# arnaucube/fhe-study

Measured on AMD Instinct MI355X. Metric: NTT/s (N=2^16, 64-bit q) per node; achieved HBM GB/s vs roofline, higher is better.
Workload: dtype u64

## Files before the change

### fhe-study_amd/binding.py

```python
import ctypes
import os
import subprocess
import sys

import numpy as np

_HERE = os.path.dirname(os.path.abspath(__file__))
LIB_PATH = os.environ.get("FHE_NTT_LIB") or os.path.join(_HERE, "libfhe_ntt.so")
CSRC = os.path.join(_HERE, "csrc")
SOURCES = ["capi.hip", "ntt_kernels.hip", "ntt_kernels_q62.hip", "ntt_persist.hip", "digit_mac.hip", "digit32.hip", "bfv32.hip", "smallq.hip", "generic63.hip", "zring.hip", "glue.hip", "tfhe_boot.hip"]
HEADERS = ["ntt_kernels.hpp", "ntt_rounds.hpp", "ntt_persist.hpp", "persist_sched.hpp", "digit_mac.hpp", "digit32.hpp", "bfv32.hpp", "smallq.hpp", "ntt32_rounds.hpp", "ntt32_big.hpp", "zq_device.hpp", "capi_internal.hpp", "mac_kernel.hpp", "ntt_kernels.hip",
           os.path.join("..", "..", "include", "fhe_ntt.h"), os.path.join("..", "..", "include", "fhe_ntt_experimental.h")]
OBJ_DIR = os.path.join(_HERE, "build")
HIPCC_FLAGS = ["--offload-arch=gfx950", "-O3", "-std=c++17", "-fPIC", "-Wno-unused-result",
               "-ffp-contract=off"]

FHE_OK = 0
FHE_E_BAD_N = -1
FHE_E_BAD_Q = -2
FHE_E_NO_ROOT = -3
FHE_E_NULL = -4
FHE_E_HIP = -5
FHE_E_NO_DEVICE = -6
FHE_E_PARAM_MISMATCH = -7
FHE_E_NOT_CANONICAL = -8
FHE_E_INVALID = -9
FHE_A_IS_EVALS, FHE_B_IS_EVALS, FHE_OUT_EVALS = 1, 2, 4

EXPORTS = [
    "fhe_ntt_plan_get", "fhe_ntt_plan_info", "fhe_ntt_plan_tables",
    "fhe_ntt_forward", "fhe_ntt_inverse", "fhe_rq_mul", "fhe_rq_mul_checked",
    "fhe_rq_pointwise_mul", "fhe_rq_check_canonical",
    "fhe_ntt_forward_dev", "fhe_ntt_inverse_dev", "fhe_rq_mul_dev",
    "fhe_rq_mul_workspace_bytes", "fhe_rq_pointwise_mul_dev", "fhe_fill_synthetic_dev",
    "fhe_ntt_set_batch_tile", "fhe_ntt_kernel_timing_enable", "fhe_ntt_kernel_timing_read",
    "fhe_ntt_kernel_timing_reset",
    "fhe_ntt_device_count", "fhe_last_error", "fhe_ntt_version", "fhe_ntt_shutdown",
    "fhe_ntt_plan_prepare", "fhe_ntt_plan_arithmetic", "fhe_ntt_set_check_canonical", "fhe_shard_range", "fhe_shard_gather_dev", "fhe_ntt_release_stream_workspace", "fhe_ntt_workspace_bytes",
    "fhe_tggsw_prepared_words", "fhe_tggsw_prepare_dev", "fhe_tggsw_external_product_prepared_dev",
    "fhe_glwe_ksk_prepared_words", "fhe_glwe_ksk_prepare_dev", "fhe_glwe_key_switch_prepared_dev",
    "fhe_bfv_rlk_prepared_words", "fhe_bfv_rlk_prepare_dev", "fhe_bfv_relinearize_prepared_dev", "fhe_bfv_mul_prepared_dev",
    "fhe_r_naive_mul", "fhe_r_naive_mul_dev", "fhe_mul_div_round_dev",
    "fhe_bfv_tensor", "fhe_bfv_tensor_dev", "fhe_bfv_relinearize_dev", "fhe_bfv_mul", "fhe_bfv_mul_dev",
    "fhe_tn_mul", "fhe_tn_mul_dev", "fhe_tggsw_external_product", "fhe_tggsw_external_product_dev",
# ... 561 lines not shown
```

### fhe-study_amd/csrc/bfv32.hip

```cpp
#include "bfv32.hpp"
#include "ntt32_big.hpp"

#include <type_traits>

namespace fhe {

__device__ __forceinline__ u32 mont32(u32 x, u32 y, u32 p, u32 pinv_neg) {
    const u64 t = (u64)x * y;
    const u32 m = (u32)t * pinv_neg;
    return (u32)((t + (u64)m * p) >> 32);
}
__device__ __forceinline__ u64 crt2(u32 rA, u32 rB, u32 pA, u32 pB, Tw32 crt) {
    const u32 rAb = csub_u32(rA, pB);
    const u32 diff = rB - rAb + pB;
    const u32 h = csub_u32(mul_shoup32(diff, crt, pB), pB);
    return (u64)rA + (u64)pA * h;
}

#ifndef FHE_B32_INV_T
#define FHE_B32_INV_T 2
#endif
#ifndef FHE_B32_INV_R
#define FHE_B32_INV_R 1
#endif
#ifndef FHE_B32_FWD_PRELOAD
#define FHE_B32_FWD_PRELOAD 1
#endif
#ifndef FHE_B32_FWD_WAVES
#define FHE_B32_FWD_WAVES 4
#endif
#ifndef FHE_B32_RELIN_WAVES
#define FHE_B32_RELIN_WAVES 4
#endif
#ifndef FHE_B32_FWD2_WAVES
#define FHE_B32_FWD2_WAVES 6
#endif
#ifndef FHE_B32_FWD2_PRELOAD
#define FHE_B32_FWD2_PRELOAD 0
#endif
#ifndef FHE_B32_FWD3_WAVES
#define FHE_B32_FWD3_WAVES 4
#endif
#ifndef FHE_B32_FWD3_RELOAD
#define FHE_B32_FWD3_RELOAD 0
#endif
constexpr int fwd_waves(int npr) { return npr == 2 ? FHE_B32_FWD2_WAVES : npr == 3 ? FHE_B32_FWD3_WAVES : FHE_B32_FWD_WAVES; }
constexpr bool fwd_reload(int npr) { return npr == 3 && FHE_B32_FWD3_RELOAD != 0; }
constexpr bool fwd_preload(int npr) { return npr == 2 ? FHE_B32_FWD2_PRELOAD != 0 : FHE_B32_FWD_PRELOAD != 0; }
#ifndef FHE_B32_PARK_LDS
#define FHE_B32_PARK_LDS 1
#endif
constexpr int kRelinWps = 4;
#ifndef FHE_B32_INV_LOOSE
#define FHE_B32_INV_LOOSE 1
#endif
template <int MODE> constexpr int last_in_of() { return (FHE_B32_INV_LOOSE && MODE != 0) ? 8 : 2; }
template <int MODE, int LB>
__device__ __forceinline__ void inv_block(u32 (&v)[1][16], u32 *lds, const Tw32 *ltw, const Tw32 *gtw, u32 tf, u32 p, u32 p2, u32 bq, u32 blk) {
    if constexpr (FHE_B32_INV_LOOSE && MODE != 0) inv_big_loose<LB, MODE == 2, last_in_of<MODE>()>(v, lds, ltw, gtw, tf, p, bq, 1u, blk);
    else if constexpr (MODE == 0) inv_big<LB>(v, lds, ltw, gtw, tf, p, p2, 1u, blk);
    else if constexpr (MODE == 1) inv_big_direct<LB, false>(v, lds, ltw, gtw, tf, p, p2, 1u, blk);
    else inv_big_direct<LB, true>(v, lds, ltw, gtw, tf, p, p2, 1u, blk);
}
template <int LB>
struct Blk {
    using C = Big32<LB>;
    static constexpr u32 M = C::M, TH = C::TH;
    static constexpr size_t LDS(int tables) { return C::TILE_BYTES + (size_t)tables * C::TW_BYTES; }
    static constexpr int park_lds(int tables, int words, int wps) {
        const long wgs = (4L * wps * 64) / (long)TH;
        const long budget = 160L * 1024 / (wgs < 1 ? 1 : wgs) - 1024;
        const long k = (budget - (long)LDS(tables)) / (8L * (long)TH);
        return k < 0 ? 0 : (k > words ? words : (int)k);
    }
    static constexpr size_t LDS_PARKED(int tables, int words, int wps) { return LDS(tables) + (size_t)park_lds(tables, words, wps) * 8 * TH; }
    static __device__ __forceinline__ Tw32 *table(unsigned char *smem, int i) { return reinterpret_cast<Tw32 *>(smem + C::TILE_BYTES + i * C::TW_BYTES); }
};

template <int LB, int NPR, bool WORD32, bool BELOWP = false>
__global__ __launch_bounds__((Big32<LB>::TH), fwd_waves(NPR)) void bfv32_forward_kernel(Bfv32Args a) {
    static_assert(!BELOWP || WORD32, "words below a 27-bit prime are below 2^32");
    using C = Big32<LB>;
    using K = Blk<LB>;
    extern __shared__ __attribute__((aligned(16))) unsigned char smem_raw[];
    u32 *lds = reinterpret_cast<u32 *>(smem_raw);
    const u32 tf = threadIdx.x;
    const u64 g8 = blockIdx.x / 16;
    const u32 r16 = blockIdx.x % 16;
    const u64 row = g8 * 8 + (r16 & 7u);
    const u32 blk = r16 >> 3;
    if (row >= a.rows) return;
#pragma unroll
    for (int i = 0; i < NPR; i++) stage_tw32_block<C::TH>(K::table(smem_raw, i), a.t.tw_fwd[NPR == 1 ? blockIdx.y : i], C::LTW_N, tf, 1u, blk);
    const u64 *__restrict__ src = a.src + row * K::M;
    typename std::conditional<WORD32, u32, u64>::type x[16];
#pragma unroll
    for (int k = 0; k < 16; k++) x[k] = (typename std::conditional<WORD32, u32, u64>::type)src[(u32)k * C::TH + tf];
    __syncthreads();
#pragma unroll
    for (int i = 0; i < NPR; i++) {
        const u32 pr = NPR == 1 ? blockIdx.y : (u32)i;
        const u32 p = a.t.p[pr], p2 = 2u * p;
        if constexpr (fwd_reload(NPR)) {
            if (i > 0) {
                u64 sa = reinterpret_cast<u64>(src);
                asm volatile("" : "+s"(sa));
                const gu64 *ps = reinterpret_cast<const gu64 *>(sa);
#pragma unroll
                for (int k = 0; k < 16; k++) x[k] = (typename std::conditional<WORD32, u32, u64>::type)ps[(u32)k * C::TH + tf];
            }
        }
        u32 v[1][16];
#pragma unroll
        for (int k = 0; k < 16; k++)
            v[0][k] = BELOWP ? (u32)x[k] : WORD32 ? csub_u32(barrett2p_32((u32)x[k], p, a.t.bq[pr]), p) : reduce64_32(x[k], p, a.t.mu[pr]);
        fwd_big<LB, 0, 1, fwd_preload(NPR)>(v, lds, K::table(smem_raw, i), a.t.tw_fwd[pr], tf, p, p2, a.t.bq[pr], 1u, blk);
        u32 *__restrict__ dst = a.fw + (((u64)pr * a.rows + row) << (LB + 1)) + blk * K::M + tf * 4u;
#pragma unroll
        for (int j = 0; j < 4; j++) {
            uint4 o;
            o.x = barrett2p_32(v[0][4 * j], p, a.t.bq[pr]); o.y = barrett2p_32(v[0][4 * j + 1], p, a.t.bq[pr]);
            o.z = barrett2p_32(v[0][4 * j + 2], p, a.t.bq[pr]); o.w = barrett2p_32(v[0][4 * j + 3], p, a.t.bq[pr]);
            *reinterpret_cast<uint4 *>(dst + j * (K::M / 4)) = o;
// ... 30 lines not shown

#ifndef FHE_B32_INT_TAIL
#define FHE_B32_INT_TAIL 1
#endif
__device__ __forceinline__ u64 zq_from_f64_small(double ef, double qf, double qinv, u32 q) {
    const double e = round(ef);
#if FHE_B32_INT_TAIL
    const double k = floor(e * qinv);
    int r = (int)fma(-k, qf, e);
    r += (r >> 31) & (int)q;
    return (u64)min((u32)r, (u32)r - q);
#else
    const double k = rint(e * qinv);
    double r = fma(-k, qf, e);
    r = r < 0.0 ? r + qf : r;
    r = r < 0.0 ? r + qf : r;
    r = r >= qf ? r - qf : r;
    return (u64)(u32)r;
#endif
}
__device__ __forceinline__ double exact_quotient(double N, double den, double rden) {
    const double q0 = N * rden;
    const double r = fma(-q0, den, N);
    return fma(r, rden, q0);
}
template <bool SMALL>
__device__ __forceinline__ u64 scale_round(const Bfv32Args &a, long long v) {
    const double N = a.numf * (double)v;
    const double x = a.rdenf != 0.0 ? exact_quotient(N, a.denf, a.rdenf) : N / a.denf;
    if constexpr (SMALL) return zq_from_f64_small(x, (double)a.q, a.qinvf, (u32)a.q);
    else return zq_from_f64_mu(a.q, a.qmu, round(x));
}

template <int LB, bool INT, bool SMALL>
__global__ __launch_bounds__((Big32<LB>::TH), 4) void bfv32_tensor_inverse_kernel(Bfv32Args a) {
    using C = Big32<LB>;
    using K = Blk<LB>;
    extern __shared__ __attribute__((aligned(16))) unsigned char smem_raw[];
    u32 *lds = reinterpret_cast<u32 *>(smem_raw);
    const u32 tf = threadIdx.x;
    const u64 g8 = blockIdx.x / 24;
    const u32 r24 = blockIdx.x % 24;
    const u64 b = g8 * 8 + (r24 & 7u);
    const u32 which = r24 >> 3;
    if (b >= a.batch) return;
#pragma unroll
    for (int i = 0; i < 4; i++) stage_tw32_block<C::TH>(K::table(smem_raw, i), a.t.tw_inv[i >> 1], C::LTW_N, tf, 1u, (u32)(i & 1));
    __syncthreads();
    auto prime = [&](auto prc) __attribute__((always_inline)) {
        constexpr int pr = decltype(prc)::value;
        const u32 p = a.t.p[pr], p2 = 2u * p, pn = a.pinv_neg[pr];
        const u32 *__restrict__ fw = a.fw + (((u64)pr * a.rows) << (LB + 1));
        auto block = [&](u32 blk, u32 (&v)[1][16]) __attribute__((always_inline)) {
            const u32 off = blk * K::M + tf * 4u;
            auto rowp = [&](u32 w) { return fw + (((u64)w * a.batch + b) << (LB + 1)) + off; };
            const u32 *__restrict__ ra = rowp(which == 2 ? 1 : 0), *__restrict__ rb = rowp(which == 0 ? 2 : 3);
            const u32 *__restrict__ rc = rowp(1), *__restrict__ rd = rowp(2);
#pragma unroll
            for (int j = 0; j < 4; j++) {
                const uint4 xa = *reinterpret_cast<const uint4 *>(ra + j * (K::M / 4)), xb = *reinterpret_cast<const uint4 *>(rb + j * (K::M / 4));
                u32 t[4] = {mont32(xa.x, xb.x, p, pn), mont32(xa.y, xb.y, p, pn), mont32(xa.z, xb.z, p, pn), mont32(xa.w, xb.w, p, pn)};
                if (which == 1) {
                    const uint4 xc = *reinterpret_cast<const uint4 *>(rc + j * (K::M / 4)), xd = *reinterpret_cast<const uint4 *>(rd + j * (K::M / 4));
                    t[0] = csub_u32(t[0] + mont32(xc.x, xd.x, p, pn), p2); t[1] = csub_u32(t[1] + mont32(xc.y, xd.y, p, pn), p2);
                    t[2] = csub_u32(t[2] + mont32(xc.z, xd.z, p, pn), p2); t[3] = csub_u32(t[3] + mont32(xc.w, xd.w, p, pn), p2);
                }
                v[0][4 * j] = t[0]; v[0][4 * j + 1] = t[1]; v[0][4 * j + 2] = t[2]; v[0][4 * j + 3] = t[3];
            }
#ifndef FHE_B32_ABLATE_INV
            inv_block<FHE_B32_INV_T, LB>(v, lds, K::table(smem_raw, 2 * pr + (int)blk), a.t.tw_inv[pr], tf, p, p2, a.t.bq[pr], blk);
#endif
        };
        u32 v0[1][16], v1[1][16];
        block(0u, v0);
        block(1u, v1);
        const Tw32 ni = a.ninv_mont[pr], w1ni = a.w1ninv_mont[pr];
        u64 parked = 0;
        u32 tfe = tf;
        asm volatile("" : "+v"(tfe));
        u64 *po = a.out + ((u64)which * a.batch + b) * K::M + tfe;
        u64 psa = reinterpret_cast<u64>(po);
        asm volatile("" : "+v"(psa));
        const gu64 *ps = reinterpret_cast<const gu64 *>(psa);
        if constexpr (pr == 1) parked = ps[0];
#pragma unroll
        for (int k = 0; k < 16; k++) {
            u32 rl = v0[0][k], rh = v1[0][k];
            last_stage<last_in_of<FHE_B32_INV_T>()>(rl, rh, ni, w1ni, p);
            if constexpr (pr == 0) {
                po[(u32)k * C::TH] = ((u64)rh << 32) | rl;
            } else {
                const u32 loA = (u32)parked, hiA = (u32)(parked >> 32);
                if (k + 1 < 16) parked = ps[(u32)(k + 1) * C::TH];
                const long long lo = (long long)crt2(loA, rl, a.t.p[0], a.t.p[1], a.t.crt);
                const long long hi = (long long)crt2(hiA, rh, a.t.p[0], a.t.p[1], a.t.crt);
#ifndef FHE_B32_ABLATE_EPI
                u64 zl, zh;
                if constexpr (INT) {
                    zl = zq_scale_round_int(a.int_num * (u64)lo, a.q, a.qmu);
                    zh = zq_scale_round_int(a.int_num * (u64)hi, a.q, a.qmu);
                } else {
                    zl = scale_round<SMALL>(a, lo);
                    zh = scale_round<SMALL>(a, hi);
                }
#else
                const u64 zl = (u64)lo, zh = (u64)hi;
#endif
                po[(u32)k * C::TH] = zl >= zh ? zl - zh : (a.q + zl) - zh;
                __builtin_amdgcn_sched_barrier(0);
            }
        }
    };
    prime(std::integral_constant<int, 0>{});
    prime(std::integral_constant<int, 1>{});
}

template <int LB, bool SMALL>
__global__ __launch_bounds__((Big32<LB>::TH), FHE_B32_RELIN_WAVES) void bfv32_relin_inverse_kernel(Bfv32Args a) {
    using C = Big32<LB>;
    using K = Blk<LB>;
    extern __shared__ __attribute__((aligned(16))) unsigned char smem_raw[];
    u32 *lds = reinterpret_cast<u32 *>(smem_raw);
    const u32 tf = threadIdx.x;
    const u64 g8 = blockIdx.x / 16;
    const u32 r16 = blockIdx.x % 16;
    const u64 b = g8 * 8 + (r16 & 7u);
    const u32 o = r16 >> 3;
    if (b >= a.batch) return;
#pragma unroll
    for (int i = 0; i < 6; i++) stage_tw32_block<C::TH>(K::table(smem_raw, i), a.t.tw_inv[i >> 1], C::LTW_N, tf, 1u, (u32)(i & 1));
    __syncthreads();
    const u64 off = ((u64)o * a.batch + b) * K::M + tf;
    u64 *park0 = a.park + off, *park1 = park0 + 2 * a.batch * K::M;
    auto prime = [&](auto prc) __attribute__((always_inline)) {
        constexpr int pr = decltype(prc)::value;
        const u32 p = a.t.p[pr], p2 = 2u * p, pn = a.pinv_neg[pr];
        auto block = [&](u32 blk, u32 (&v)[1][16]) __attribute__((always_inline)) {
            const u32 bo = blk * K::M + tf * 4u;
            const u32 *__restrict__ rx = a.x + (((u64)pr * a.batch + b) << (LB + 1)) + bo;
            const u32 *__restrict__ rk = a.key + (((u64)pr * 2 + o) << (LB + 1)) + bo;
#pragma unroll
            for (int j = 0; j < 4; j++) {
                const uint4 xa = *reinterpret_cast<const uint4 *>(rx + j * (K::M / 4)), xb = *reinterpret_cast<const uint4 *>(rk + j * (K::M / 4));
                v[0][4 * j] = mont32(xa.x, xb.x, p, pn); v[0][4 * j + 1] = mont32(xa.y, xb.y, p, pn);
                v[0][4 * j + 2] = mont32(xa.z, xb.z, p, pn); v[0][4 * j + 3] = mont32(xa.w, xb.w, p, pn);
            }
#ifndef FHE_B32_ABLATE_INV
            inv_block<FHE_B32_INV_R, LB>(v, lds, K::table(smem_raw, 2 * pr + (int)blk), a.t.tw_inv[pr], tf, p, p2, a.t.bq[pr], blk);
#endif
        };
        u32 v0[1][16], v1[1][16];
        block(0u, v0);
        block(1u, v1);
        const Tw32 ni = a.ninv_mont[pr], w1ni = a.w1ninv_mont[pr];
        u64 pk0 = 0, pk1 = 0;
        u64 psa0 = reinterpret_cast<u64>(park0), psa1 = reinterpret_cast<u64>(park1);
        asm volatile("" : "+v"(psa0), "+v"(psa1));
        const gu64 *ps0 = reinterpret_cast<const gu64 *>(psa0), *ps1 = reinterpret_cast<const gu64 *>(psa1);
        constexpr int KL = FHE_B32_PARK_LDS ? K::park_lds(6, 16, kRelinWps) : 0;
        u64 *lpark = reinterpret_cast<u64 *>(smem_raw + K::LDS(6)) + tf;
// ... 56 lines not shown
bool bfv32_shape_supported(uint64_t q, uint64_t n, uint64_t pq) {
    if (n < 1024 || n > 8192 || (n & (n - 1)) || q < 2) return false;
    const unsigned ln = bits_of64(n - 1), bq = bits_of64(q - 1);
    if (2 * bq + ln + 1 > 54) return false;
    if (pq && (pq < q || bq + bits_of64(pq - 1) + ln > 82)) return false;
    return true;
}

template <typename K>
static hipError_t launch_big(K kernel, const char *name, int lp, size_t lds, unsigned th, u64 grid, const Bfv32Args &a, hipStream_t st,
                             unsigned gridy = 1) {
    if (grid == 0) return hipSuccess;
    if (grid > 0x7fffffffull) return hipErrorInvalidValue;
    if (hipError_t e = allow_big_lds((const void *)kernel, lds)) return e;
    KernelTimer kt(name, lp, st);
    hipLaunchKernelGGL(kernel, dim3((unsigned)grid, gridy), dim3(th), lds, st, a);
    return hipGetLastError();
}
#define FHE_BIG_SWITCH(KERNEL, NAME, GRID, GRIDY, TABLES, PARKW, WPS)                                                               \
    switch (a.log_n2) {                                                                                                      \
        case 11: return launch_big(KERNEL<10>, NAME, 11, Blk<10>::LDS_PARKED(TABLES, PARKW, WPS), Big32<10>::TH, GRID, a, st, GRIDY); \
        case 12: return launch_big(KERNEL<11>, NAME, 12, Blk<11>::LDS_PARKED(TABLES, PARKW, WPS), Big32<11>::TH, GRID, a, st, GRIDY); \
        case 13: return launch_big(KERNEL<12>, NAME, 13, Blk<12>::LDS_PARKED(TABLES, PARKW, WPS), Big32<12>::TH, GRID, a, st, GRIDY); \
        case 14: return launch_big(KERNEL<13>, NAME, 14, Blk<13>::LDS_PARKED(TABLES, PARKW, WPS), Big32<13>::TH, GRID, a, st, GRIDY); \
    }                                                                                                                        \
    return hipErrorNotSupported;

template <int LB> static constexpr auto bfv32_forward2 = bfv32_forward_kernel<LB, 2, true>;
template <int LB> static constexpr auto bfv32_forward3 = bfv32_forward_kernel<LB, 3, true>;
template <int LB> static constexpr auto bfv32_forward2b = bfv32_forward_kernel<LB, 2, true, true>;
template <int LB> static constexpr auto bfv32_forward3b = bfv32_forward_kernel<LB, 3, true, true>;
template <int LB> static constexpr auto bfv32_forward1w = bfv32_forward_kernel<LB, 1, false>;
hipError_t launch_bfv32_forward(const Bfv32Args &a, hipStream_t st) {
    const u64 grid = 16 * ((a.rows + 7) / 8);
    if (a.primes == 2 && a.word32 && a.below_p) { FHE_BIG_SWITCH(bfv32_forward2b, "bfv32_forward", grid, 1, 2, 0, 4) }
    if (a.primes == 3 && a.word32 && a.below_p) { FHE_BIG_SWITCH(bfv32_forward3b, "bfv32_forward3", grid, 1, 3, 0, 4) }
    if (a.primes == 2 && a.word32) { FHE_BIG_SWITCH(bfv32_forward2, "bfv32_forward", grid, 1, 2, 0, 4) }
    if (a.primes == 3 && a.word32) { FHE_BIG_SWITCH(bfv32_forward3, "bfv32_forward3", grid, 1, 3, 0, 4) }
    if (a.primes == 3) { FHE_BIG_SWITCH(bfv32_forward1w, "bfv32_forward_key", grid, 3, 1, 0, 4) }
    return hipErrorNotSupported;
}
template <int LB> static constexpr auto bfv32_tensor_inverse_f64 = bfv32_tensor_inverse_kernel<LB, false, false>;
template <int LB> static constexpr auto bfv32_tensor_inverse_f64s = bfv32_tensor_inverse_kernel<LB, false, true>;
template <int LB> static constexpr auto bfv32_tensor_inverse_int = bfv32_tensor_inverse_kernel<LB, true, false>;
hipError_t launch_bfv32_tensor_inverse(const Bfv32Args &a, hipStream_t st) {
    if (a.int_num) { FHE_BIG_SWITCH(bfv32_tensor_inverse_int, "bfv32_tensor_inverse", 24 * ((a.batch + 7) / 8), 1, 4, 0, 4) }
    if (a.small_f64) { FHE_BIG_SWITCH(bfv32_tensor_inverse_f64s, "bfv32_tensor_inverse", 24 * ((a.batch + 7) / 8), 1, 4, 0, 4) }
    FHE_BIG_SWITCH(bfv32_tensor_inverse_f64, "bfv32_tensor_inverse", 24 * ((a.batch + 7) / 8), 1, 4, 0, 4)
}
template <int LB> static constexpr auto bfv32_relin_inverse_gen = bfv32_relin_inverse_kernel<LB, false>;
template <int LB> static constexpr auto bfv32_relin_inverse_small = bfv32_relin_inverse_kernel<LB, true>;
hipError_t launch_bfv32_relin_inverse(const Bfv32Args &a, hipStream_t st) {
    if (a.small_f64) { FHE_BIG_SWITCH(bfv32_relin_inverse_small, "bfv32_relin_inverse", 16 * ((a.batch + 7) / 8), 1, 6, (FHE_B32_PARK_LDS ? 16 : 0), kRelinWps) }
    FHE_BIG_SWITCH(bfv32_relin_inverse_gen, "bfv32_relin_inverse", 16 * ((a.batch + 7) / 8), 1, 6, (FHE_B32_PARK_LDS ? 16 : 0), kRelinWps)
}
#undef FHE_BIG_SWITCH

bool bfv32_ablated() {
#if defined(FHE_B32_ABLATE_INV) || defined(FHE_B32_ABLATE_EPI)
    return true;
#else
    return false;
#endif
}

}
```

### fhe-study_amd/csrc/bfv32.hpp

```cpp
#pragma once
#include "digit32.hpp"

namespace fhe {

struct Bfv32Args {
    Ext32Args t;
    uint32_t pinv_neg[3];
    Tw32 ninv_mont[3];
    Tw32 w1ninv_mont[3];
    uint32_t log_n2;
    const u64 *src;
    uint32_t *fw;
    u64 rows;
    uint32_t primes;
    uint32_t word32;
    uint32_t below_p;
    const uint32_t *x, *key;
    const u64 *addend;
    u64 *out;
    u64 *park;
    u64 batch, q;
    u64 qmu;
    double numf, denf;
    double rdenf;
    u64 int_num;
    uint32_t small_f64;
    double qinvf;
};

bool bfv32_shape_supported(uint64_t q, uint64_t n, uint64_t pq);
hipError_t launch_bfv32_forward(const Bfv32Args &a, hipStream_t st);
hipError_t launch_bfv32_tensor_inverse(const Bfv32Args &a, hipStream_t st);
hipError_t launch_bfv32_relin_inverse(const Bfv32Args &a, hipStream_t st);

}
```

### fhe-study_amd/csrc/zring.hip

```cpp
#include <cstdio>
#include <cstdlib>
#include <cstring>
#include <map>
#include <vector>

#include "capi_internal.hpp"
#include "digit_mac.hpp"
#include "digit32.hpp"
#include "bfv32.hpp"
#include "ntt_rounds.hpp"
#include "zq_device.hpp"
#include "mac_kernel.hpp"

using fhe::Mod;
using fhe::Tw;
using fhe::u32;
using fhe::u64;
typedef unsigned __int128 u128;

static const u64 kCrtPrimes[3] = {
    2305843009211596801ull,
    2305843009196916737ull,
    2305843009146585089ull,
};
// ... 443 lines not shown

static bool bfv32_on(uint64_t q, uint64_t n, uint64_t pq) { return fhe_ext32_enabled() && fhe::bfv32_shape_supported(q, n, pq); }
static int bfv32_args(uint64_t n, fhe::Bfv32Args *a) {
    int rc = fhe_ext32_tables(2 * n, &a->t);
    if (rc != FHE_OK) return rc;
    a->log_n2 = ceil_log2(2 * n);
    for (int i = 0; i < 3; i++) {
        const uint32_t p = a->t.p[i];
        uint32_t inv = p;
        for (int it = 0; it < 5; it++) inv *= 2u - p * inv;
        a->pinv_neg[i] = 0u - inv;
        const u64 w = ((u64)a->t.ninv[i].w << 32) % p;
        a->ninv_mont[i] = fhe::Tw32{(uint32_t)w, (uint32_t)((w << 32) / p)};
        const fhe_ntt_plan *plan = nullptr;
        if ((rc = fhe_ntt_plan_get(p, 2 * n, &plan)) != FHE_OK) return rc;
        const u64 w1 = (plan->roots_inv[1] * w) % p;
        a->w1ninv_mont[i] = fhe::Tw32{(uint32_t)w1, (uint32_t)((w1 << 32) / p)};
    }
    return FHE_OK;
}
static bool bfv32_small_f64_on() {
    static const bool on = [] { const char *e = getenv("FHE_BFV_SMALL_F64"); return !(e && e[0] == '0'); }();
    return on;
}
static double bfv32_rden(uint64_t den) {
    static const bool on = [] { const char *e = getenv("FHE_BFV_FAST_DIV"); return !(e && e[0] == '0'); }();
    return (on && (den & 1ull) && den < (1ull << 48)) ? 1.0 / (double)den : 0.0;
}
static uint32_t bfv32_below_p(uint64_t q, const fhe::Bfv32Args &a, int primes) {
    static const bool on = [] { const char *e = getenv("FHE_BFV_BELOW_P"); return !(e && e[0] == '0'); }();
    for (int i = 0; i < primes; i++) if (q > a.t.p[i]) return 0u;
    return on ? 1u : 0u;
}
static int bfv32_tensor(uint64_t q, uint64_t n, uint64_t t, const void *d_ab, void *d_c, size_t batch, hipStream_t st) {
    fhe::Bfv32Args a{};
    int rc = bfv32_args(n, &a);
    if (rc != FHE_OK) return rc;
    void *wsv = nullptr;
    if ((rc = fhe_workspace_get(1, (u64)2 * 4 * batch * 2 * n * 4, st, &wsv)) != FHE_OK) return rc;
    a.src = (const u64 *)d_ab; a.fw = (uint32_t *)wsv; a.rows = 4 * (u64)batch; a.primes = 2; a.word32 = 1;
    a.below_p = bfv32_below_p(q, a, 2);
    if (a.below_p && (rc = fhe_check_canonical_words(q, d_ab, 4 * batch * n, st, "fhe_bfv_tensor_dev")) != FHE_OK) return rc;
    hipError_t e = fhe::launch_bfv32_forward(a, st);
    if (e != hipSuccess) return fhe_hip_fail(e, "bfv32_forward_kernel");
    a.batch = batch; a.out = (u64 *)d_c; a.q = q; a.qmu = ~0ull / q; a.numf = (double)t; a.denf = (double)q;
    a.rdenf = ((unsigned __int128)2 * n * (q - 1) * (q - 1) * t / q < ((unsigned __int128)1 << 52)) ? bfv32_rden(q) : 0.0;
    {
        static const bool on = [] { const char *e = getenv("FHE_BFV_INT_ROUND"); return e && e[0] == '1'; }();
        const unsigned __int128 vmax = (unsigned __int128)2 * n * (q - 1) * (q - 1);
        a.int_num = (on && t != 0 && vmax * t < ((unsigned __int128)1 << 52)) ? t : 0;
        a.small_f64 = (bfv32_small_f64_on() && q < (1ull << 30) && vmax * t / q < ((unsigned __int128)1 << 50)) ? 1u : 0u;
        a.qinvf = 1.0 / (double)q;
    }
    e = fhe::launch_bfv32_tensor_inverse(a, st);
    return e == hipSuccess ? FHE_OK : fhe_hip_fail(e, "bfv32_tensor_inverse_kernel");
}
static int bfv32_rlk_prepare(uint64_t n, const u64 *d_rlk, void *prep, hipStream_t st) {
    fhe::Bfv32Args a{};
    int rc = bfv32_args(n, &a);
    if (rc != FHE_OK) return rc;
    a.src = d_rlk; a.fw = (uint32_t *)prep; a.rows = 2; a.primes = 3;
    hipError_t e = fhe::launch_bfv32_forward(a, st);
    return e == hipSuccess ? FHE_OK : fhe_hip_fail(e, "bfv32_forward_kernel");
}
static int bfv32_relinearize(uint64_t q, uint64_t n, uint64_t pq, const void *d_prep, const void *d_c, void *d_out, size_t batch,
                             hipStream_t st) {
    fhe::Bfv32Args a{};
    int rc = bfv32_args(n, &a);
    if (rc != FHE_OK) return rc;
    void *wsv = nullptr;
    const u64 x_bytes = (u64)3 * batch * 2 * n * 4, park_bytes = (u64)2 * 2 * batch * n * 8;
    if ((rc = fhe_workspace_get(1, x_bytes + park_bytes, st, &wsv)) != FHE_OK) return rc;
    a.park = (u64 *)((unsigned char *)wsv + x_bytes);
    a.src = (const u64 *)d_c + 2 * (u64)batch * n; a.fw = (uint32_t *)wsv; a.rows = batch; a.primes = 3; a.word32 = 1;
    a.below_p = bfv32_below_p(q, a, 3);
    if (a.below_p && (rc = fhe_check_canonical_words(q, a.src, batch * n, st, "fhe_bfv_relinearize_dev (c2)")) != FHE_OK) return rc;
    hipError_t e = fhe::launch_bfv32_forward(a, st);
    if (e != hipSuccess) return fhe_hip_fail(e, "bfv32_forward_kernel");
    a.x = (const uint32_t *)wsv; a.key = (const uint32_t *)d_prep;
    a.addend = (const u64 *)d_c; a.out = (u64 *)d_out; a.batch = batch; a.q = q; a.qmu = ~0ull / q; a.numf = 1.0; a.denf = (double)(pq / q);
    a.rdenf = (pq % q == 0 && pq / q >= (1ull << 12)) ? bfv32_rden(pq / q) : 0.0;
    a.small_f64 = (bfv32_small_f64_on() && q < (1ull << 30) && pq / q >= (1ull << 14)) ? 1u : 0u;
    a.qinvf = 1.0 / (double)q;
    e = fhe::launch_bfv32_relin_inverse(a, st);
    return e == hipSuccess ? FHE_OK : fhe_hip_fail(e, "bfv32_relin_inverse_kernel");
}

extern "C" int fhe_bfv_tensor_dev(uint64_t q, uint64_t n, uint64_t t, const void *d_ab, void *d_c, size_t batch,
                                  void *hip_stream) {
    int rc = check_pow2_n(n, "fhe_bfv_tensor_dev");
    if (rc != FHE_OK) return rc;
    if (q < 2 || (q >> 63)) return fhe_fail(FHE_E_BAD_Q, "fhe_bfv_tensor_dev: q must be in [2, 2^63)");
    if (batch == 0) return FHE_OK;
    if (!d_ab || !d_c) return fhe_fail(FHE_E_NULL, "fhe_bfv_tensor_dev: NULL buffer");
    REQUIRE_ALIGNED(d_ab); REQUIRE_ALIGNED(d_c);
    if (bfv32_on(q, n, 0)) return bfv32_tensor(q, n, t, d_ab, d_c, batch, (hipStream_t)hip_stream);
    const u64 n2 = 2 * n;
    ZCtx z;
    rc = zctx_init(&z, n2, primes_for_bits(2 * bits_of(q - 1) + ceil_log2(n) + 1, false));
    if (rc != FHE_OK) return rc;
    hipStream_t st = (hipStream_t)hip_stream;
    const u64 words = batch * n2;
    void *wsv = nullptr;
    rc = fhe_workspace_get(1, (4 + 3 * (size_t)z.K) * words * 8, st, &wsv);
    if (rc != FHE_OK) return rc;
    u64 *AB = (u64 *)wsv, *R = AB + 4 * words;
    for (int k = 0; k < z.K; k++) {
        if ((rc = z_forward_src(z, k, (const u64 *)d_ab, AB, 4 * batch, n, st)) != FHE_OK) return rc;
        u64 *Rk = R + 3 * (u64)k * words;
        { fhe::KernelTimer kt_("zr_tensor", 0, st);
        hipLaunchKernelGGL(fhe::zr_tensor_kernel, dim3(fhe_ew_grid(words)), dim3(256), 0, st, (const u64 *)AB, Rk, words, z.cc.m[k]);
        }
// ... 104 lines not shown
    if (bfv32_on(q, n, pq)) return bfv32_relinearize(q, n, pq, d_prepared, d_c, d_out, batch, (hipStream_t)hip_stream);
    return bfv_relinearize_with(z, h, q, n, pq, (const u64 *)d_prepared, d_c, d_out, batch, (hipStream_t)hip_stream);
}

extern "C" int fhe_bfv_relinearize_dev(uint64_t q, uint64_t n, uint64_t pq, const void *d_rlk, const void *d_c,
                                       void *d_out, size_t batch, void *hip_stream) {
    ZCtx z;
    unsigned h = 0;
    int rc = bfv_relin_ctx(&z, &h, q, n, pq, "fhe_bfv_relinearize_dev");
    if (rc != FHE_OK) return rc;
    if (batch == 0) return FHE_OK;
    if (!d_rlk || !d_c || !d_out) return fhe_fail(FHE_E_NULL, "fhe_bfv_relinearize_dev: NULL buffer");
    REQUIRE_ALIGNED(d_rlk); REQUIRE_ALIGNED(d_c); REQUIRE_ALIGNED(d_out);
    hipStream_t st = (hipStream_t)hip_stream;
    const size_t tensor_words = 3 * batch * n;
    void *w0 = nullptr;
    if ((rc = fhe_workspace_get(0, (tensor_words + 16 * n) * 8, st, &w0)) != FHE_OK) return rc;
    u64 *prep = (u64 *)w0 + tensor_words;
    if (bfv32_on(q, n, pq)) {
        if ((rc = bfv32_rlk_prepare(n, (const u64 *)d_rlk, prep, st)) != FHE_OK) return rc;
        return bfv32_relinearize(q, n, pq, prep, d_c, d_out, batch, st);
    }
    if ((rc = bfv_rlk_prepare(z, h, n, (const u64 *)d_rlk, prep, prep + 12 * n, st)) != FHE_OK) return rc;
    return bfv_relinearize_with(z, h, q, n, pq, prep, d_c, d_out, batch, st);
}

static int bfv_mul_common(uint64_t q, uint64_t n, uint64_t t, uint64_t pq, const void *d_rlk, bool prepared, const void *d_ab,
                          void *d_out, size_t batch, void *hip_stream) {
    if (batch == 0) return FHE_OK;
    const size_t kw = 16 * (size_t)n;
    void *c = nullptr;
    int rc = fhe_workspace_get(0, (3 * batch * n + kw) * 8, (hipStream_t)hip_stream, &c);
    if (rc != FHE_OK) return rc;
    rc = fhe_bfv_tensor_dev(q, n, t, d_ab, c, batch, hip_stream);
    if (rc != FHE_OK) return rc;
    return prepared ? fhe_bfv_relinearize_prepared_dev(q, n, pq, d_rlk, c, d_out, batch, hip_stream)
                    : fhe_bfv_relinearize_dev(q, n, pq, d_rlk, c, d_out, batch, hip_stream);
}

extern "C" int fhe_bfv_mul_dev(uint64_t q, uint64_t n, uint64_t t, uint64_t pq, const void *d_rlk, const void *d_ab,
                               void *d_out, size_t batch, void *hip_stream) {
    return bfv_mul_common(q, n, t, pq, d_rlk, false, d_ab, d_out, batch, hip_stream);
}
extern "C" int fhe_bfv_mul_prepared_dev(uint64_t q, uint64_t n, uint64_t t, uint64_t pq, const void *d_prepared, const void *d_ab,
                                        void *d_out, size_t batch, void *hip_stream) {
    return bfv_mul_common(q, n, t, pq, d_prepared, true, d_ab, d_out, batch, hip_stream);
}

extern "C" int fhe_tn_mul_dev(uint64_t n, const void *d_a, const void *d_b, void *d_out, size_t batch,
                              void *hip_stream) {
    int rc = check_pow2_n(n, "fhe_tn_mul_dev");
    if (rc != FHE_OK) return rc;
    if (batch == 0) return FHE_OK;
    if (!d_a || !d_b || !d_out) return fhe_fail(FHE_E_NULL, "fhe_tn_mul_dev: NULL buffer");
    REQUIRE_ALIGNED(d_a); REQUIRE_ALIGNED(d_b); REQUIRE_ALIGNED(d_out);
    ZCtx z;
    rc = zctx_init(&z, n, primes_for_bits(128 + ceil_log2(n), true));
    if (rc != FHE_OK) return rc;
    hipStream_t st = (hipStream_t)hip_stream;
    const u64 words = batch * n;
    void *wsv = nullptr;
    rc = fhe_workspace_get(1, (2 + (size_t)z.K) * words * 8, st, &wsv);
    if (rc != FHE_OK) return rc;
    u64 *A = (u64 *)wsv, *B = A + words, *R = B + words;
    for (int k = 0; k < z.K; k++) {
        if ((rc = z_forward_src(z, k, (const u64 *)d_a, A, batch, n, st)) != FHE_OK) return rc;
// ... 451 lines not shown
```

Baseline: 2.789 million.

## Fuse BFV c2 forward NTT into tensor-inverse kernel, skipping separate relin forward pass

In the BFV multiply path, the workgroup that produces the c2 component of the tensor now keeps it in LDS and immediately runs the three-prime forward NTT. It writes the transformed words straight into the relinearization workspace, so the separate relin forward kernel and the c2 round-trip through HBM go away. Workgroup indexing is moved into a shared helper header, with c2 slots scheduled first so the longer work starts early. The fused variant uses more LDS (six twiddle tables) and a different occupancy target, and the c2 workgroups take longer than the others, which can cause load imbalance. The metric is NTT throughput, and this BFV multiply path may not be what is measured.

```diff
diff --git a/fhe-study_amd/binding.py b/fhe-study_amd/binding.py
--- a/fhe-study_amd/binding.py
+++ b/fhe-study_amd/binding.py
@@ -9,7 +9,7 @@
 LIB_PATH = os.environ.get("FHE_NTT_LIB") or os.path.join(_HERE, "libfhe_ntt.so")
 CSRC = os.path.join(_HERE, "csrc")
 SOURCES = ["capi.hip", "ntt_kernels.hip", "ntt_kernels_q62.hip", "ntt_persist.hip", "digit_mac.hip", "digit32.hip", "bfv32.hip", "smallq.hip", "generic63.hip", "zring.hip", "glue.hip", "tfhe_boot.hip"]
-HEADERS = ["ntt_kernels.hpp", "ntt_rounds.hpp", "ntt_persist.hpp", "persist_sched.hpp", "digit_mac.hpp", "digit32.hpp", "bfv32.hpp", "smallq.hpp", "ntt32_rounds.hpp", "ntt32_big.hpp", "zq_device.hpp", "capi_internal.hpp", "mac_kernel.hpp", "ntt_kernels.hip",
+HEADERS = ["ntt_kernels.hpp", "ntt_rounds.hpp", "ntt_persist.hpp", "persist_sched.hpp", "digit_mac.hpp", "digit32.hpp", "bfv32.hpp", "bfv32_index.hpp", "smallq.hpp", "ntt32_rounds.hpp", "ntt32_big.hpp", "zq_device.hpp", "capi_internal.hpp", "mac_kernel.hpp", "ntt_kernels.hip",
            os.path.join("..", "..", "include", "fhe_ntt.h"), os.path.join("..", "..", "include", "fhe_ntt_experimental.h")]
 OBJ_DIR = os.path.join(_HERE, "build")
 HIPCC_FLAGS = ["--offload-arch=gfx950", "-O3", "-std=c++17", "-fPIC", "-Wno-unused-result",
diff --git a/fhe-study_amd/csrc/bfv32.hip b/fhe-study_amd/csrc/bfv32.hip
--- a/fhe-study_amd/csrc/bfv32.hip
+++ b/fhe-study_amd/csrc/bfv32.hip
@@ -1,4 +1,5 @@
 #include "bfv32.hpp"
+#include "bfv32_index.hpp"
 #include "ntt32_big.hpp"
 
 #include <type_traits>
@@ -47,10 +48,17 @@
 constexpr int fwd_waves(int npr) { return npr == 2 ? FHE_B32_FWD2_WAVES : npr == 3 ? FHE_B32_FWD3_WAVES : FHE_B32_FWD_WAVES; }
 constexpr bool fwd_reload(int npr) { return npr == 3 && FHE_B32_FWD3_RELOAD != 0; }
 constexpr bool fwd_preload(int npr) { return npr == 2 ? FHE_B32_FWD2_PRELOAD != 0 : FHE_B32_FWD_PRELOAD != 0; }
+#ifndef FHE_B32_FUSE_WAVES
+#define FHE_B32_FUSE_WAVES 6
+#endif
+constexpr int tensor_waves(int lb, bool fuse) { return fuse && lb == 13 ? FHE_B32_FUSE_WAVES : 4; }
+#ifndef FHE_B32_FUSE_PRELOAD
+#define FHE_B32_FUSE_PRELOAD 0
+#endif
 #ifndef FHE_B32_PARK_LDS
 #define FHE_B32_PARK_LDS 1
 #endif
-constexpr int kRelinWps = 4;
+constexpr int kRelinWps = FHE_B32_RELIN_WAVES;
 #ifndef FHE_B32_INV_LOOSE
 #define FHE_B32_INV_LOOSE 1
 #endif
@@ -85,10 +93,9 @@
     extern __shared__ __attribute__((aligned(16))) unsigned char smem_raw[];
     u32 *lds = reinterpret_cast<u32 *>(smem_raw);
     const u32 tf = threadIdx.x;
-    const u64 g8 = blockIdx.x / 16;
-    const u32 r16 = blockIdx.x % 16;
-    const u64 row = g8 * 8 + (r16 & 7u);
-    const u32 blk = r16 >> 3;
+    const Bfv32Wg wg = bfv32_wg<2>(blockIdx.x);
+    const u64 row = wg.unit;
+    const u32 blk = wg.slot;
     if (row >= a.rows) return;
 #pragma unroll
     for (int i = 0; i < NPR; i++) stage_tw32_block<C::TH>(K::table(smem_raw, i), a.t.tw_fwd[NPR == 1 ? blockIdx.y : i], C::LTW_N, tf, 1u, blk);
@@ -185,17 +192,17 @@
     else return zq_from_f64_mu(a.q, a.qmu, round(x));
 }
 
-template <int LB, bool INT, bool SMALL>
-__global__ __launch_bounds__((Big32<LB>::TH), 4) void bfv32_tensor_inverse_kernel(Bfv32Args a) {
+template <int LB, bool INT, bool SMALL, bool FUSE>
+__global__ __launch_bounds__((Big32<LB>::TH), tensor_waves(LB, FUSE)) void bfv32_tensor_inverse_kernel(Bfv32Args a) {
     using C = Big32<LB>;
     using K = Blk<LB>;
     extern __shared__ __attribute__((aligned(16))) unsigned char smem_raw[];
     u32 *lds = reinterpret_cast<u32 *>(smem_raw);
     const u32 tf = threadIdx.x;
-    const u64 g8 = blockIdx.x / 24;
-    const u32 r24 = blockIdx.x % 24;
-    const u64 b = g8 * 8 + (r24 & 7u);
-    const u32 which = r24 >> 3;
+    const Bfv32Wg wg = bfv32_tensor_wg<FUSE>(blockIdx.x);
+    const u64 b = wg.unit;
+    const u32 which = wg.slot;
+    const bool c2_here = FUSE && which == 2;
     if (b >= a.batch) return;
 #pragma unroll
     for (int i = 0; i < 4; i++) stage_tw32_block<C::TH>(K::table(smem_raw, i), a.t.tw_inv[i >> 1], C::LTW_N, tf, 1u, (u32)(i & 1));
@@ -236,6 +243,7 @@
         asm volatile("" : "+v"(psa));
         const gu64 *ps = reinterpret_cast<const gu64 *>(psa);
         if constexpr (pr == 1) parked = ps[0];
+        if constexpr (FUSE && pr == 1) { if (c2_here) __syncthreads(); }
 #pragma unroll
         for (int k = 0; k < 16; k++) {
             u32 rl = v0[0][k], rh = v1[0][k];
@@ -259,13 +267,42 @@
 #else
                 const u64 zl = (u64)lo, zh = (u64)hi;
 #endif
-                po[(u32)k * C::TH] = zl >= zh ? zl - zh : (a.q + zl) - zh;
+                const u64 z = zl >= zh ? zl - zh : (a.q + zl) - zh;
+                if (c2_here) lds[(u32)k * C::TH + tf] = (u32)z;
+                else po[(u32)k * C::TH] = z;
                 __builtin_amdgcn_sched_barrier(0);
             }
         }
     };
     prime(std::integral_constant<int, 0>{});
     prime(std::integral_constant<int, 1>{});
+    if constexpr (FUSE) {
+        if (!c2_here) return;
+        __syncthreads();
+#pragma unroll
+        for (int i = 0; i < 6; i++) stage_tw32_block<C::TH>(K::table(smem_raw, i), a.t.tw_fwd[i >> 1], C::LTW_N, tf, 1u, (u32)(i & 1));
+        u32 x[16];
+#pragma unroll
+        for (int k = 0; k < 16; k++) x[k] = lds[(u32)k * C::TH + tf];
+        __syncthreads();
+#pragma unroll 1
+        for (u32 i = 0; i < 6; i++) {
+            const u32 pr = i >> 1, blk = i & 1u;
+            const u32 p = a.t.p[pr], p2 = 2u * p, bq = a.t.bq[pr];
+            u32 v[1][16];
+#pragma unroll
+            for (int k = 0; k < 16; k++) v[0][k] = x[k];
+            fwd_big<LB, 0, 1, FHE_B32_FUSE_PRELOAD != 0>(v, lds, K::table(smem_raw, (int)i), a.t.tw_fwd[pr], tf, p, p2, bq, 1u, blk);
+            u32 *__restrict__ dst = a.xfw + (((u64)pr * a.batch + b) << (LB + 1)) + blk * K::M + tf * 4u;
+#pragma unroll
+            for (int j = 0; j < 4; j++) {
+                uint4 o;
+                o.x = barrett2p_32(v[0][4 * j], p, bq); o.y = barrett2p_32(v[0][4 * j + 1], p, bq);
+                o.z = barrett2p_32(v[0][4 * j + 2], p, bq); o.w = barrett2p_32(v[0][4 * j + 3], p, bq);
+                *reinterpret_cast<uint4 *>(dst + j * (K::M / 4)) = o;
+            }
+        }
+    }
 }
 
 template <int LB, bool SMALL>
@@ -275,10 +312,9 @@
     extern __shared__ __attribute__((aligned(16))) unsigned char smem_raw[];
     u32 *lds = reinterpret_cast<u32 *>(smem_raw);
     const u32 tf = threadIdx.x;
-    const u64 g8 = blockIdx.x / 16;
-    const u32 r16 = blockIdx.x % 16;
-    const u64 b = g8 * 8 + (r16 & 7u);
-    const u32 o = r16 >> 3;
+    const Bfv32Wg wg = bfv32_wg<2>(blockIdx.x);
+    const u64 b = wg.unit;
+    const u32 o = wg.slot;
     if (b >= a.batch) return;
 #pragma unroll
     for (int i = 0; i < 6; i++) stage_tw32_block<C::TH>(K::table(smem_raw, i), a.t.tw_inv[i >> 1], C::LTW_N, tf, 1u, (u32)(i & 1));
@@ -401,7 +437,7 @@
 template <int LB> static constexpr auto bfv32_forward3b = bfv32_forward_kernel<LB, 3, true, true>;
 template <int LB> static constexpr auto bfv32_forward1w = bfv32_forward_kernel<LB, 1, false>;
 hipError_t launch_bfv32_forward(const Bfv32Args &a, hipStream_t st) {
-    const u64 grid = 16 * ((a.rows + 7) / 8);
+    const u64 grid = bfv32_grid<2>(a.rows);
     if (a.primes == 2 && a.word32 && a.below_p) { FHE_BIG_SWITCH(bfv32_forward2b, "bfv32_forward", grid, 1, 2, 0, 4) }
     if (a.primes == 3 && a.word32 && a.below_p) { FHE_BIG_SWITCH(bfv32_forward3b, "bfv32_forward3", grid, 1, 3, 0, 4) }
     if (a.primes == 2 && a.word32) { FHE_BIG_SWITCH(bfv32_forward2, "bfv32_forward", grid, 1, 2, 0, 4) }
@@ -409,19 +445,28 @@
     if (a.primes == 3) { FHE_BIG_SWITCH(bfv32_forward1w, "bfv32_forward_key", grid, 3, 1, 0, 4) }
     return hipErrorNotSupported;
 }
-template <int LB> static constexpr auto bfv32_tensor_inverse_f64 = bfv32_tensor_inverse_kernel<LB, false, false>;
-template <int LB> static constexpr auto bfv32_tensor_inverse_f64s = bfv32_tensor_inverse_kernel<LB, false, true>;
-template <int LB> static constexpr auto bfv32_tensor_inverse_int = bfv32_tensor_inverse_kernel<LB, true, false>;
+template <int LB> static constexpr auto bfv32_tensor_inverse_f64 = bfv32_tensor_inverse_kernel<LB, false, false, false>;
+template <int LB> static constexpr auto bfv32_tensor_inverse_f64s = bfv32_tensor_inverse_kernel<LB, false, true, false>;
+template <int LB> static constexpr auto bfv32_tensor_inverse_int = bfv32_tensor_inverse_kernel<LB, true, false, false>;
+template <int LB> static constexpr auto bfv32_tensor_fwd3_f64 = bfv32_tensor_inverse_kernel<LB, false, false, true>;
+template <int LB> static constexpr auto bfv32_tensor_fwd3_f64s = bfv32_tensor_inverse_kernel<LB, false, true, true>;
+template <int LB> static constexpr auto bfv32_tensor_fwd3_int = bfv32_tensor_inverse_kernel<LB, true, false, true>;
 hipError_t launch_bfv32_tensor_inverse(const Bfv32Args &a, hipStream_t st) {
-    if (a.int_num) { FHE_BIG_SWITCH(bfv32_tensor_inverse_int, "bfv32_tensor_inverse", 24 * ((a.batch + 7) / 8), 1, 4, 0, 4) }
-    if (a.small_f64) { FHE_BIG_SWITCH(bfv32_tensor_inverse_f64s, "bfv32_tensor_inverse", 24 * ((a.batch + 7) / 8), 1, 4, 0, 4) }
-    FHE_BIG_SWITCH(bfv32_tensor_inverse_f64, "bfv32_tensor_inverse", 24 * ((a.batch + 7) / 8), 1, 4, 0, 4)
+    const u64 grid = bfv32_grid<3>(a.batch);
+    if (a.xfw) {
+        if (a.int_num) { FHE_BIG_SWITCH(bfv32_tensor_fwd3_int, "bfv32_tensor_inverse_fwd3", grid, 1, 6, 0, 4) }
+        if (a.small_f64) { FHE_BIG_SWITCH(bfv32_tensor_fwd3_f64s, "bfv32_tensor_inverse_fwd3", grid, 1, 6, 0, 4) }
+        FHE_BIG_SWITCH(bfv32_tensor_fwd3_f64, "bfv32_tensor_inverse_fwd3", grid, 1, 6, 0, 4)
+    }
+    if (a.int_num) { FHE_BIG_SWITCH(bfv32_tensor_inverse_int, "bfv32_tensor_inverse", grid, 1, 4, 0, 4) }
+    if (a.small_f64) { FHE_BIG_SWITCH(bfv32_tensor_inverse_f64s, "bfv32_tensor_inverse", grid, 1, 4, 0, 4) }
+    FHE_BIG_SWITCH(bfv32_tensor_inverse_f64, "bfv32_tensor_inverse", grid, 1, 4, 0, 4)
 }
 template <int LB> static constexpr auto bfv32_relin_inverse_gen = bfv32_relin_inverse_kernel<LB, false>;
 template <int LB> static constexpr auto bfv32_relin_inverse_small = bfv32_relin_inverse_kernel<LB, true>;
 hipError_t launch_bfv32_relin_inverse(const Bfv32Args &a, hipStream_t st) {
-    if (a.small_f64) { FHE_BIG_SWITCH(bfv32_relin_inverse_small, "bfv32_relin_inverse", 16 * ((a.batch + 7) / 8), 1, 6, (FHE_B32_PARK_LDS ? 16 : 0), kRelinWps) }
-    FHE_BIG_SWITCH(bfv32_relin_inverse_gen, "bfv32_relin_inverse", 16 * ((a.batch + 7) / 8), 1, 6, (FHE_B32_PARK_LDS ? 16 : 0), kRelinWps)
+    if (a.small_f64) { FHE_BIG_SWITCH(bfv32_relin_inverse_small, "bfv32_relin_inverse", bfv32_grid<2>(a.batch), 1, 6, (FHE_B32_PARK_LDS ? 16 : 0), kRelinWps) }
+    FHE_BIG_SWITCH(bfv32_relin_inverse_gen, "bfv32_relin_inverse", bfv32_grid<2>(a.batch), 1, 6, (FHE_B32_PARK_LDS ? 16 : 0), kRelinWps)
 }
 #undef FHE_BIG_SWITCH
 
diff --git a/fhe-study_amd/csrc/bfv32.hpp b/fhe-study_amd/csrc/bfv32.hpp
--- a/fhe-study_amd/csrc/bfv32.hpp
+++ b/fhe-study_amd/csrc/bfv32.hpp
@@ -18,6 +18,7 @@
     const uint32_t *x, *key;
     const u64 *addend;
     u64 *out;
+    uint32_t *xfw;
     u64 *park;
     u64 batch, q;
     u64 qmu;
diff --git a/fhe-study_amd/csrc/bfv32_index.hpp b/fhe-study_amd/csrc/bfv32_index.hpp
--- /dev/null
+++ b/fhe-study_amd/csrc/bfv32_index.hpp
@@ -0,0 +1,28 @@
+#pragma once
+#include <cstdint>
+
+#if defined(__HIPCC__)
+#define FHE_IDX_HD __host__ __device__
+#else
+#define FHE_IDX_HD
+#endif
+
+namespace fhe {
+
+struct Bfv32Wg {
+    uint64_t unit;
+    uint32_t slot;
+};
+template <int S>
+FHE_IDX_HD constexpr uint64_t bfv32_grid(uint64_t units) { return (uint64_t)(8 * S) * ((units + 7) / 8); }
+template <int S>
+FHE_IDX_HD constexpr Bfv32Wg bfv32_wg(uint64_t id) {
+    return Bfv32Wg{(id / (8 * S)) * 8 + (id % 8), (uint32_t)((id % (8 * S)) / 8)};
+}
+template <bool C2FIRST>
+FHE_IDX_HD constexpr Bfv32Wg bfv32_tensor_wg(uint64_t id) {
+    const Bfv32Wg w = bfv32_wg<3>(id);
+    return Bfv32Wg{w.unit, C2FIRST ? 2u - w.slot : w.slot};
+}
+
+}
diff --git a/fhe-study_amd/csrc/zring.hip b/fhe-study_amd/csrc/zring.hip
--- a/fhe-study_amd/csrc/zring.hip
+++ b/fhe-study_amd/csrc/zring.hip
@@ -499,12 +499,19 @@
     for (int i = 0; i < primes; i++) if (q > a.t.p[i]) return 0u;
     return on ? 1u : 0u;
 }
-static int bfv32_tensor(uint64_t q, uint64_t n, uint64_t t, const void *d_ab, void *d_c, size_t batch, hipStream_t st) {
+static bool bfv32_fuse_c2_on(uint64_t q, uint64_t n, uint64_t pq) {
+    static const bool on = [] { const char *e = getenv("FHE_BFV_FUSE_C2"); return !(e && e[0] == '0'); }();
+    return on && bfv32_on(q, n, pq) && q <= fhe::kExt32PrimeC && q <= fhe::kExt32PrimeB && q <= fhe::kExt32PrimeA;
+}
+static u64 bfv32_fw_bytes(uint64_t n, size_t batch) { return (u64)2 * 4 * batch * 2 * n * 4; }
+static u64 bfv32_x_bytes(uint64_t n, size_t batch) { return (u64)3 * batch * 2 * n * 4; }
+static int bfv32_tensor(uint64_t q, uint64_t n, uint64_t t, const void *d_ab, void *d_c, size_t batch, hipStream_t st, bool fuse_c2 = false) {
     fhe::Bfv32Args a{};
     int rc = bfv32_args(n, &a);
     if (rc != FHE_OK) return rc;
     void *wsv = nullptr;
-    if ((rc = fhe_workspace_get(1, (u64)2 * 4 * batch * 2 * n * 4, st, &wsv)) != FHE_OK) return rc;
+    if ((rc = fhe_workspace_get(1, bfv32_fw_bytes(n, batch) + (fuse_c2 ? bfv32_x_bytes(n, batch) : 0), st, &wsv)) != FHE_OK) return rc;
+    if (fuse_c2) a.xfw = (uint32_t *)((unsigned char *)wsv + bfv32_fw_bytes(n, batch));
     a.src = (const u64 *)d_ab; a.fw = (uint32_t *)wsv; a.rows = 4 * (u64)batch; a.primes = 2; a.word32 = 1;
     a.below_p = bfv32_below_p(q, a, 2);
     if (a.below_p && (rc = fhe_check_canonical_words(q, d_ab, 4 * batch * n, st, "fhe_bfv_tensor_dev")) != FHE_OK) return rc;
@@ -531,20 +538,28 @@
     return e == hipSuccess ? FHE_OK : fhe_hip_fail(e, "bfv32_forward_kernel");
 }
 static int bfv32_relinearize(uint64_t q, uint64_t n, uint64_t pq, const void *d_prep, const void *d_c, void *d_out, size_t batch,
-                             hipStream_t st) {
+                             hipStream_t st, bool c2_transformed = false) {
     fhe::Bfv32Args a{};
     int rc = bfv32_args(n, &a);
     if (rc != FHE_OK) return rc;
     void *wsv = nullptr;
-    const u64 x_bytes = (u64)3 * batch * 2 * n * 4, park_bytes = (u64)2 * 2 * batch * n * 8;
-    if ((rc = fhe_workspace_get(1, x_bytes + park_bytes, st, &wsv)) != FHE_OK) return rc;
-    a.park = (u64 *)((unsigned char *)wsv + x_bytes);
-    a.src = (const u64 *)d_c + 2 * (u64)batch * n; a.fw = (uint32_t *)wsv; a.rows = batch; a.primes = 3; a.word32 = 1;
-    a.below_p = bfv32_below_p(q, a, 3);
-    if (a.below_p && (rc = fhe_check_canonical_words(q, a.src, batch * n, st, "fhe_bfv_relinearize_dev (c2)")) != FHE_OK) return rc;
-    hipError_t e = fhe::launch_bfv32_forward(a, st);
-    if (e != hipSuccess) return fhe_hip_fail(e, "bfv32_forward_kernel");
-    a.x = (const uint32_t *)wsv; a.key = (const uint32_t *)d_prep;
+    const u64 x_bytes = bfv32_x_bytes(n, batch), park_bytes = (u64)2 * 2 * batch * n * 8;
+    hipError_t e = hipSuccess;
+    if (c2_transformed) {
+        if ((rc = fhe_workspace_get(1, bfv32_fw_bytes(n, batch) + x_bytes, st, &wsv)) != FHE_OK) return rc;
+        a.park = (u64 *)wsv;
+        a.x = (const uint32_t *)((unsigned char *)wsv + bfv32_fw_bytes(n, batch));
+    } else {
+        if ((rc = fhe_workspace_get(1, x_bytes + park_bytes, st, &wsv)) != FHE_OK) return rc;
+        a.park = (u64 *)((unsigned char *)wsv + x_bytes);
+        a.src = (const u64 *)d_c + 2 * (u64)batch * n; a.fw = (uint32_t *)wsv; a.rows = batch; a.primes = 3; a.word32 = 1;
+        a.below_p = bfv32_below_p(q, a, 3);
+        if (a.below_p && (rc = fhe_check_canonical_words(q, a.src, batch * n, st, "fhe_bfv_relinearize_dev (c2)")) != FHE_OK) return rc;
+        e = fhe::launch_bfv32_forward(a, st);
+        if (e != hipSuccess) return fhe_hip_fail(e, "bfv32_forward_kernel");
+        a.x = (const uint32_t *)wsv;
+    }
+    a.key = (const uint32_t *)d_prep;
     a.addend = (const u64 *)d_c; a.out = (u64 *)d_out; a.batch = batch; a.q = q; a.qmu = ~0ull / q; a.numf = 1.0; a.denf = (double)(pq / q);
     a.rdenf = (pq % q == 0 && pq / q >= (1ull << 12)) ? bfv32_rden(pq / q) : 0.0;
     a.small_f64 = (bfv32_small_f64_on() && q < (1ull << 30) && pq / q >= (1ull << 14)) ? 1u : 0u;
@@ -715,6 +730,21 @@
     void *c = nullptr;
     int rc = fhe_workspace_get(0, (3 * batch * n + kw) * 8, (hipStream_t)hip_stream, &c);
     if (rc != FHE_OK) return rc;
+    if (bfv32_fuse_c2_on(q, n, pq)) {
+        hipStream_t st = (hipStream_t)hip_stream;
+        if (!d_ab) return fhe_fail(FHE_E_NULL, "fhe_bfv_tensor_dev: NULL buffer");
+        REQUIRE_ALIGNED(d_ab);
+        if (!d_rlk || !d_out) return fhe_fail(FHE_E_NULL, "%s: NULL buffer", prepared ? "fhe_bfv_relinearize_prepared_dev" : "fhe_bfv_relinearize_dev");
+        REQUIRE_ALIGNED(d_rlk); REQUIRE_ALIGNED(d_out);
+        const void *prep = d_rlk;
+        if (!prepared) {
+            u64 *p = (u64 *)c + 3 * batch * n;
+            if ((rc = bfv32_rlk_prepare(n, (const u64 *)d_rlk, p, st)) != FHE_OK) return rc;
+            prep = p;
+        }
+        if ((rc = bfv32_tensor(q, n, t, d_ab, c, batch, st, true)) != FHE_OK) return rc;
+        return bfv32_relinearize(q, n, pq, prep, c, d_out, batch, st, true);
+    }
     rc = fhe_bfv_tensor_dev(q, n, t, d_ab, c, batch, hip_stream);
     if (rc != FHE_OK) return rc;
     return prepared ? fhe_bfv_relinearize_prepared_dev(q, n, pq, d_rlk, c, d_out, batch, hip_stream)
```

New measurement: 2.789 million (median of 2 runs). About the same (+0.0%).
